# openai/baselines

Hardware: NVIDIA H100
Metric: PPO2 learner env-steps/sec (higher is better)
Workload: dtype f16 operands / f32 accumulate (GAE f64 carry)

## Files before the change

baselines_b200/common/policies.py:

```python
import numpy as np
import torch

from .. import _lib, nn, ops
from . import spaces


RECURRENT_NETWORKS = ("lstm", "cnn_lstm")


class PolicyBuilder:

    def __init__(self, ob_space, ac_space, network, value_network=None, normalize_observations=False,
                 **network_kwargs):
        if callable(network) and not isinstance(network, str):
            raise NotImplementedError("custom network callables build TF graphs in the reference; this learner "
                                      "supports the registry names 'cnn', 'mlp', 'conv_only', 'lstm', 'cnn_lstm'")
        if network in ("lnlstm", "cnn_lnlstm") or (network in RECURRENT_NETWORKS and network_kwargs.get("layer_norm")):
            raise NotImplementedError(f"network={network!r}: layer-normalised LSTMs are not implemented "
                                      "(supported recurrent networks: 'lstm', 'cnn_lstm' without layer_norm)")
        if network in ("impala_cnn", "impala_cnn_lstm"):
            raise NotImplementedError(f"network={network!r}: the IMPALA residual tower is not implemented")
        if value_network not in (None, "shared", "copy"):
            raise NotImplementedError("value_network must be None/'shared'/'copy' (policies.py:154-166)")
        if value_network == "copy" and network in RECURRENT_NETWORKS:
# ... 247 lines not shown
        if self.pd in ("cat", "mcat"):
            ops.cat_step(self.pi_out, self.ld_pi, self.nout, self.v_out, self.ld_v, actions, values, neglogp, B,
                         uniforms=noise, seed=seed, offset_dev=self.rng_ctr, seg_off=self.seg_off)
        elif self.pd == "bern":
            ops.bern_step(self.pi_out, self.ld_pi, self.nout, self.v_out, self.ld_v, actions, values, neglogp, B,
                          uniforms=noise, seed=seed, offset_dev=self.rng_ctr)
        else:
            ops.gauss_step(self.pi_out, self.ld_pi, self.logstd, self.nout, self.v_out, self.ld_v, actions, values,
                           neglogp, B, normals=noise, seed=seed, offset_dev=self.rng_ctr)
        ops.counter_add(self.rng_ctr, 1)

    def _fused_first_wgrad(self, B, alpha):
        tp, tv = self.tower_pi, self.tower_vf
        a, b = tp.fcs[0], tv.fcs[0]
        N2, x, ldx = 2 * a.N, tp._mlp_in, 2 * tp.in_pad
        bn = 256 if N2 == 256 else (128 if N2 > 64 else 64)
        tiles = -(-a.K // 128) * -(-N2 // bn)
        kb = -(-B // 64)
        split = max(1, min(kb // 2 if kb >= 2 else 1, -(-2 * ops.num_sms() // tiles)))
        self.g0cat.zero_()
        for xs in ((x, x[:, a.Kp:]) if a.split_in else (x,)):
            ops.gemm(xs, self.dz0cat, self.g0cat, M=a.K, N=N2, K=B, lda=ldx, ldb=N2, ldc=N2, mn_major=True,
                     mode=ops.MODE_F32_ATOMIC, alpha=alpha * a.in_scale, split_k=split, tag="wgrad.pi+vf/mlp_fc0")
        a.gw.add_(self.g0cat[:, :a.N])
        b.gw.add_(self.g0cat[:, a.N:])
        ops.colsum(tp.dzfc[0], a.gb, B, a.N, N2, alpha=alpha)
        ops.colsum(tv.dzfc[0], b.gb, B, b.N, N2, alpha=alpha)

    def loss_backward(self, x, B, src_idx, actions, returns, old_values, old_neglogp, cliprange, ent_coef, vf_coef,
                      inv_M, seq=None):
        clip_dev = self.clip_dev if cliprange is None else None
        cliprange = 0.0 if cliprange is None else cliprange
        _lib.phase = "@train"
        self.forward(x, B, src_idx, seq=seq)
        if self.pd in ("cat", "mcat"):
            ops.cat_loss(self.pi_out, self.ld_pi, self.nout, self.v_out, self.ld_v, actions, src_idx, returns,
                         old_values, old_neglogp, self.adv_st, cliprange, ent_coef, vf_coef, self.dpi, self.ld_dpi,
                         self.dv, self.ld_dv, self.stats, B, cliprange_dev=clip_dev, seg_off=self.seg_off)
# ... 28 lines not shown
```

baselines_b200/csrc/conv_shift.cu:

```cuda
#include <stdlib.h>

#include <type_traits>

#include "common.cuh"
#include "tc_common.cuh"

namespace b200rl {

static constexpr int SH_BM = 128;
static constexpr int SH_CONSUMER_WARPS = 8;
static constexpr int SH_TMA_WARP = SH_CONSUMER_WARPS;
__host__ __device__ constexpr int sh_threads(bool u8) { return (SH_CONSUMER_WARPS + 1) * 32 + (u8 ? 256 : 0); }
static constexpr int SH_MAX_TAPS = 16;
__host__ __device__ constexpr int sh_arows(int KH) { return KH == 1 ? 160 : 144; }
__host__ __device__ constexpr int sh_stages(int KH) { return KH == 1 ? 6 : 4; }
static constexpr int SH_U8_STAGES = 12;
static constexpr int SH_U8_WRES_BYTES = 16 * 1024;
__host__ __device__ constexpr int sh_wgrad_krows(bool u8) { return u8 ? 128 : 64; }
__host__ __device__ constexpr int sh_wres_bytes(int KH, bool u8) {
  return u8 ? SH_U8_WRES_BYTES : KH == 1 ? 80 * 1024 : 64 * 1024;
}
static constexpr int SH_BAR_BYTES = 512;
__host__ __device__ constexpr int sh_mask_stage_bytes(int BN, bool DACT) { return DACT ? SH_BM * BN / 8 : 0; }
static constexpr int SH_EPI_WARP_BYTES = 16 * 64;
static constexpr int SH_EPI_BYTES = SH_CONSUMER_WARPS * SH_EPI_WARP_BYTES;
static constexpr int SH_WROWS_K = 96;
static constexpr int SH_WABYTES = SH_WROWS_K * 128;
__host__ __device__ constexpr int sh_wgrad_qw(int BN, int KH, bool u8) { return u8 ? 2 : BN == 32 ? 4 : KH == 1 ? 3 : 2; }

static constexpr int SH_ORDER_BAR = 2;
__device__ __forceinline__ void order_wait(int wg) {
  asm volatile("bar.sync %0, %1;" ::"r"(SH_ORDER_BAR + wg), "n"(SH_CONSUMER_WARPS * 32) : "memory");
}
__device__ __forceinline__ void order_pass(int wg) {
  asm volatile("bar.arrive %0, %1;" ::"r"(SH_ORDER_BAR + 1 - wg), "n"(SH_CONSUMER_WARPS * 32) : "memory");
}

struct AddrMap {
  int mode;
  long long sN, sY, sX;
  int Cq, s;
  int Cq_log2, s_log2;
};

__device__ __forceinline__ long long map_rowbase(const AddrMap& a, int n, int y, int x) {
  if (a.mode == 2) {
    const int sm = a.s - 1;
    return (long long)n * a.sN + (long long)(y >> a.s_log2) * a.sY + (long long)(x >> a.s_log2) * a.sX +
           ((((y & sm) << a.s_log2) + (x & sm)) << a.Cq_log2);
  }
  if (a.mode == 1) return (long long)n * a.sN + ((long long)y << a.s_log2) * a.sY + ((long long)x << a.s_log2) * a.sX;
// ... 152 lines not shown
  int Hg, Wg;
  int N;
  int taps;
  int shift[SH_MAX_TAPS];
  int min_shift;
  int vy, vx;
  __half* out;
  AddrMap omap;
  uint16_t* bits_out;
  const uint16_t* saved_bits;
  const float* bias;
  int act, dact;
  float alpha;
  int num_tiles;
};

__device__ __forceinline__ void stmatrix_x4(uint32_t addr, const uint32_t (&r)[4]) {
  asm volatile("stmatrix.sync.aligned.m8n8.x4.shared.b16 [%0], {%1, %2, %3, %4};" ::"r"(addr), "r"(r[0]), "r"(r[1]),
               "r"(r[2]), "r"(r[3])
               : "memory");
}
__device__ __forceinline__ uint4 ld_shared_v4(uint32_t addr) {
  uint4 v;
  asm volatile("ld.shared.v4.b32 {%0,%1,%2,%3}, [%4];" : "=r"(v.x), "=r"(v.y), "=r"(v.z), "=r"(v.w) : "r"(addr) : "memory");
  return v;
}
__device__ __forceinline__ void st_global_v4(void* p, const uint4& v) {
  asm volatile("st.global.v4.b32 [%0], {%1,%2,%3,%4};" ::"l"(p), "r"(v.x), "r"(v.y), "r"(v.z), "r"(v.w) : "memory");
}
__device__ __forceinline__ uint32_t h2_bits(__half2 h) { return *reinterpret_cast<const uint32_t*>(&h); }
__device__ __forceinline__ uint32_t mask_pair(uint32_t b8, int k) {
  const uint32_t b = b8 >> (2 * k);
  return ((b & 1u) | ((b & 2u) << 15)) * 0xffffu;
}

template <int BN, int KH, bool DACT, bool U8>
__global__ void __launch_bounds__(sh_threads(U8), 1)
conv_shift_fwd_kernel(const __grid_constant__ CUtensorMap tmX, const __grid_constant__ CUtensorMap tmW,
                      const __grid_constant__ ShiftParams p) {
  constexpr int SH_ABYTES = sh_arows(KH) * 128;
  constexpr int STAGE_BYTES = KH * SH_ABYTES;
  constexpr int STAGES = U8 ? SH_U8_STAGES : sh_stages(KH);
  using Ring = U8Ring<SH_BM, STAGES>;
  constexpr bool PINGPONG = !(BN == 128 && !DACT);
  constexpr int MH = PINGPONG ? 2 : 1;
  static_assert(PINGPONG || !U8, "the uint8 ring's release rule assumes ping-pong");
  constexpr int A_PITCH = U8 ? SH_BM * 128 : STAGE_BYTES;
  constexpr int A_TOTAL = U8 ? Ring::BYTES : STAGES * STAGE_BYTES;
  extern __shared__ uint8_t smem_raw[];
// ... 77 lines not shown
    }
  } else if (U8 && warp > SH_TMA_WARP) {
    u8_ring_producer<SH_BM, STAGES, 2>(p.u8, p.M, (long long)tile_first * SH_BM + p.min_shift, tile_count, smem,
                                       full_bar, head_bar, empty_bar, warp - (SH_TMA_WARP + 1), lane);
  } else {
    const int wg = __shfl_sync(0xffffffffu, warp >> 2, 0), t = threadIdx.x & 127;
    const int row0 = PINGPONG ? 0 : wg * 64;
    const uint32_t w_base = smem_u32(wres);
    const float lo = (p.act == ACT_RELU) ? 0.0f : -INFINITY;
    const __half2 lo2 = __floats2half2_rn(lo, lo);
    const __half2 zero2 = __floats2half2_rn(0.0f, 0.0f);
    const int er = lane & 15, ep = lane >> 4;
    const int erow = row0 + 16 * (warp & 3) + er;
    uint32_t epi_addr[2];
#pragma unroll
    for (int jj = 0; jj < 2; ++jj)
      epi_addr[jj] = smem_u32(sepi + warp * SH_EPI_WARP_BYTES) + er * 64 + (((2 * jj + ep) ^ ((er >> 1) & 3)) << 4);
    const bool masked = DACT && p.saved_bits != nullptr;
    float acc[MH][BN / 2];
    mbar_wait(w_bar, 0);
    for (int i = PINGPONG ? wg : 0; i < tile_count; i += PINGPONG ? 2 : 1) {
      const int tile = tile_first + i * tile_stride;
      const int s = i % STAGES, s1 = (s + 1 == STAGES) ? 0 : s + 1;
      const uint32_t ph = (uint32_t)(i / STAGES) & 1u;
      mbar_wait(&full_bar[s], ph);
      if (U8) mbar_wait(&head_bar[s1], s1 == 0 ? ph ^ 1 : ph);
      if (PINGPONG && i > 0) order_wait(wg);
      const uint32_t a_base = smem_u32(smem + s * A_PITCH) + (uint32_t)(row0 * 128);
      wgmma_fence();
#pragma unroll 1
      for (int a = 0; a < p.taps; ++a) {
        const uint32_t at = a_base + (uint32_t)p.shift[a] * 128u;
// ... 549 lines not shown
```

baselines_b200/csrc/gemm_wgmma.cu:

```cuda
#include <stdarg.h>
#include <stdio.h>
#include <stdlib.h>

#include <map>
#include <mutex>

#include "common.cuh"
#include "tc_common.cuh"

namespace b200rl {

static constexpr int BM = 128;
static constexpr int BK = 64;
static constexpr int MMA_K = 16;
static constexpr int CONSUMER_WARPS = 8;
static constexpr int NUM_THREADS = CONSUMER_WARPS * 32 + 32;


struct ConvCoords {
  int OW, OH;
  int stride_w, stride_h;
  int lower_w, lower_h;
  int S, taps;
};
// ... 19 lines not shown
  int rm_C, rm_OW, rm_Wg;
  float* ws;
};

template <int BN>
struct Cfg {
  static constexpr int A_BYTES = BM * BK * 2;
  static constexpr int B_BYTES = BN * BK * 2;
  static constexpr int STAGE_BYTES = A_BYTES + B_BYTES;
  static constexpr int STAGES_RAW = (196 * 1024) / STAGE_BYTES;
  static constexpr int STAGES = STAGES_RAW > 8 ? 8 : STAGES_RAW;
  static constexpr int SMEM_BYTES = STAGES * STAGE_BYTES + 1024  + 256 ;
};

static constexpr int BRES_STAGES = 7;
static constexpr int BRES_B_BYTES = 80 * 1024;

__device__ __forceinline__ void gemm_epi_pair(const GemmParams& p, int mode, int split, int row, int col, float v0,
                                              float v1, bool two) {
  if (mode == MODE_F32_ATOMIC) {
    if (p.ws) {
      float* w = p.ws + ((long long)split * p.M + row) * p.N + col;
      w[0] = v0;
      if (two) w[1] = v1;
      return;
    }
    float* out = reinterpret_cast<float*>(p.C) + (long long)row * p.ldc + col;
    atomicAdd(out, v0);
    if (two) atomicAdd(out + 1, v1);
    return;
// ... 41 lines not shown
  }
  int ocol = col;
  if (p.rm_C > 0) {
    const int pix = col / p.rm_C;
    ocol = ((pix / p.rm_OW) * p.rm_Wg + pix % p.rm_OW) * p.rm_C + col % p.rm_C;
  }
  __half* out = C + (long long)row * p.ldc + ocol;
  if (two && p.vec32) {
    *reinterpret_cast<__half2*>(out) = __floats2half2_rn(v0, v1);
  } else {
    out[0] = __float2half_rn(v0);
    if (two) out[1] = __float2half_rn(v1);
  }
}

template <int BN, int CPT, bool MN_MAJOR, bool IM2COL, bool BRES, int TMODE>
__global__ void __launch_bounds__(NUM_THREADS, 1)
gemm_wgmma_kernel(const __grid_constant__ CUtensorMap tmA, const __grid_constant__ CUtensorMap tmB,
                  const GemmParams p) {
  using C_ = Cfg<BN>;
  static_assert(!BRES || (IM2COL && !MN_MAJOR), "resident weights: K-major implicit conv only");
  constexpr int STAGES = BRES ? BRES_STAGES : C_::STAGES;
  constexpr int STAGE_BYTES = BRES ? C_::A_BYTES : C_::STAGE_BYTES;
  constexpr int BROWB = MN_MAJOR ? (BN >= 64 ? 128 : BN * 2) : 0;
  constexpr uint32_t LAYOUT_B = sdesc_layout(BROWB);
  constexpr int BCHUNKS = (BN >= 64) ? BN / 64 : 1;
  constexpr int TPS = BK / CPT;
  constexpr int ROWB = CPT * 2;
  constexpr uint32_t LAYOUT_A = sdesc_layout(ROWB);
  constexpr int A_SUB = BM * ROWB;
  constexpr int B_SUB = BN * ROWB;
  constexpr int A_CHUNK = BK * ROWB;
  constexpr int MCH = BM / CPT;
  extern __shared__ uint8_t smem_raw[];
  uint8_t* smem = reinterpret_cast<uint8_t*>((reinterpret_cast<uintptr_t>(smem_raw) + 1023) & ~uintptr_t(1023));
  uint8_t* bres = smem + STAGES * STAGE_BYTES;
  constexpr int ZT_BYTES = (IM2COL && !MN_MAJOR) ? B_SUB : 0;
  uint8_t* zero_tile = bres + (BRES ? BRES_B_BYTES : 0);
  uint64_t* bars = reinterpret_cast<uint64_t*>(zero_tile + ZT_BYTES);
  uint64_t* full_bar = bars;
  uint64_t* empty_bar = bars + STAGES;
  uint64_t* bres_bar = bars + 2 * STAGES;

  const int warp = threadIdx.x >> 5;
  const int lane = threadIdx.x & 31;
  const int total_work = p.m_tiles * p.n_tiles * p.splits;

  if (threadIdx.x == 0) {
    for (int s = 0; s < STAGES; ++s) {
      mbar_init(&full_bar[s], 1);
      mbar_init(&empty_bar[s], CONSUMER_WARPS);
    }
    mbar_init(bres_bar, 1);
    fence_barrier_init();
  }
  __syncthreads();

  if (warp == CONSUMER_WARPS) {
    if (elect_one()) {
      tma_prefetch_desc(&tmA);
      tma_prefetch_desc(&tmB);
      if (BRES) {
        mbar_arrive_expect_tx(bres_bar, (uint32_t)p.cv.taps * B_SUB);
        for (int g = 0; g < p.cv.taps; ++g) tma_load_2d(bres + g * B_SUB, &tmB, bres_bar, g * CPT, 0);
      }
    }
// ... 55 lines not shown
                                     (uint16_t)(g / p.cv.S));
                } else {
                  tma_load_2d(sa + j * A_CHUNK, &tmA, &full_bar[s], m_tile * BM + j * CPT, kb * BK);
                }
              }
            }
#pragma unroll
            for (int j = 0; j < BCHUNKS; ++j)
              tma_load_2d(sb + j * (BK * BROWB), &tmB, &full_bar[s], n_tile * BN + j * 64, kb * BK);
          }
        }
        __syncwarp();
        if (++s == STAGES) { s = 0; ph ^= 1; }
      }
    }
  } else {
    const int wg = warp >> 2;
    const int t = threadIdx.x & 127;
    const int mode = (TMODE >= 0) ? TMODE : p.mode;
    float acc[BN / 2];
    int s = 0;
    uint32_t ph = 0;
    if (ZT_BYTES > 0) {
      for (int i = threadIdx.x; i < ZT_BYTES / 16; i += CONSUMER_WARPS * 32)
        reinterpret_cast<uint4*>(zero_tile)[i] = make_uint4(0u, 0u, 0u, 0u);
      fence_proxy_async_smem();
      asm volatile("bar.sync 1, %0;" ::"n"(CONSUMER_WARPS * 32) : "memory");
    }
    if (BRES) mbar_wait(bres_bar, 0);
    for (int work = blockIdx.x; work < total_work; work += gridDim.x) {
// ... 193 lines not shown
      const long long r = i / cols;
      out[r * ldo + (i - r * cols)] += t;
    }
    __syncthreads();
  }
}

int sum_partials(const float* ws, int parts, long long rows, int cols, float* out, long long ldo, cudaStream_t stream) {
  const long long n = rows * cols;
  long long blocks = (n + 31) / 32;
  if (blocks > 16LL * num_sms()) blocks = 16LL * num_sms();
  sum_partials_kernel<<<(int)blocks, 256, 0, stream>>>(ws, parts, rows, cols, out, ldo);
  return check_launch("sum_partials_kernel");
}

template <int BN, int CPT, bool MN, bool IM2COL, bool BRES = false, int TMODE = -1>
static int launch(const CUtensorMap& tmA, const CUtensorMap& tmB, const GemmParams& p, int max_ctas,
                  cudaStream_t stream) {
  using C_ = Cfg<BN>;
  constexpr int ZT = (IM2COL && !MN) ? BN * CPT * 2 : 0;
  constexpr int SMEM = (BRES ? (BRES_STAGES * C_::A_BYTES + BRES_B_BYTES + 1024 + 256) : C_::SMEM_BYTES) + ZT;
  static_assert(SMEM <= 227 * 1024, "gemm: shared memory budget");
  static bool attr_set = false;
  auto kern = gemm_wgmma_kernel<BN, CPT, MN, IM2COL, BRES, TMODE>;
  if (!attr_set) {
    cudaError_t e = cudaFuncSetAttribute(kern, cudaFuncAttributeMaxDynamicSharedMemorySize, SMEM);
    if (e != cudaSuccess) {
      set_last_error("cudaFuncSetAttribute(smem=%d): %s", SMEM, cudaGetErrorString(e));
      return B200RL_ERR_CUDA;
    }
    attr_set = true;
  }
  const int total = p.m_tiles * p.n_tiles * p.splits;
  int grid = total < num_sms() ? total : num_sms();
  if (max_ctas > 0 && grid > max_ctas) grid = max_ctas;
  kern<<<grid, NUM_THREADS, SMEM, stream>>>(tmA, tmB, p);
  return check_launch("gemm_wgmma_kernel");
}

static void fill_splits(GemmParams& p, int split_k) {
  int splits = split_k < 1 ? 1 : split_k;
  if (splits > p.kb_total) splits = p.kb_total;
  p.kb_per_split = ceil_div(p.kb_total, splits);
  p.splits = ceil_div(p.kb_total, p.kb_per_split);
}

static int gemm_dispatch(int BN, int mn_major, int mode, const CUtensorMap& tmA, const CUtensorMap& tmB,
                         const GemmParams& p, int max_ctas, cudaStream_t stream) {
  if (mn_major) {
    B200RL_REQUIRE(mode == MODE_F32_ATOMIC, "gemm: the MN-major (wgrad) layout uses the fp32 atomic epilogue");
    if (BN == 64) return launch<64, 64, true, false, false, MODE_F32_ATOMIC>(tmA, tmB, p, max_ctas, stream);
    if (BN == 256) return launch<256, 64, true, false, false, MODE_F32_ATOMIC>(tmA, tmB, p, max_ctas, stream);
    return launch<128, 64, true, false, false, MODE_F32_ATOMIC>(tmA, tmB, p, max_ctas, stream);
  }
#define GEMM_KMAJOR(bn)                                                                                         \
  switch (mode) {                                                                                               \
    case MODE_F16_ACT: return launch<bn, 64, false, false, false, MODE_F16_ACT>(tmA, tmB, p, max_ctas, stream);   \
    case MODE_F32_STORE: return launch<bn, 64, false, false, false, MODE_F32_STORE>(tmA, tmB, p, max_ctas, stream); \
    case MODE_F16_DACT: return launch<bn, 64, false, false, false, MODE_F16_DACT>(tmA, tmB, p, max_ctas, stream);  \
    default: return launch<bn, 64, false, false, false, MODE_F32_ATOMIC>(tmA, tmB, p, max_ctas, stream);          \
  }
  switch (BN) {
    case 32: GEMM_KMAJOR(32)
    case 64: GEMM_KMAJOR(64)
    case 128: GEMM_KMAJOR(128)
    default: GEMM_KMAJOR(256)
  }
#undef GEMM_KMAJOR
}

template <int CPT, bool MN>
static int launch_conv(int BN, bool bres, const CUtensorMap& tmA, const CUtensorMap& tmB, const GemmParams& p,
                       cudaStream_t st) {
  if (MN) {
    switch (BN) {
      case 32: return launch<32, CPT, MN, true>(tmA, tmB, p, 0, st);
      case 64: return launch<64, CPT, MN, true>(tmA, tmB, p, 0, st);
      case 128: return launch<128, CPT, MN, true>(tmA, tmB, p, 0, st);
      default: break;
    }
  } else if (bres) {
// ... 28 lines not shown
  B200RL_REQUIRE(rm_C == 0 || (rm_C % 16 == 0 && rm_OW > 0 && rm_Wg >= rm_OW && (mode == MODE_F16_ACT || mode == MODE_F16_DACT)),
                 "gemm: bad column remap");
  B200RL_REQUIRE(M > 0 && N > 0 && K > 0, "gemm: bad shape M=%d N=%d K=%d", M, N, K);
  B200RL_REQUIRE((lda % 8) == 0 && (ldb % 8) == 0, "gemm: lda/ldb must be multiples of 8 fp16 (16 B): %lld %lld", lda,
                 ldb);
  B200RL_REQUIRE((reinterpret_cast<uintptr_t>(A) & 15) == 0 && (reinterpret_cast<uintptr_t>(B) & 15) == 0,
                 "gemm: operands must be 16-byte aligned");
  B200RL_REQUIRE(mode >= 0 && mode <= 3, "gemm: bad mode %d", mode);
  B200RL_REQUIRE(mode != MODE_F16_DACT || saved != nullptr || saved_bits != nullptr,
                 "gemm: MODE_F16_DACT needs the saved activation (or its bit mask)");
  B200RL_REQUIRE(saved_bits == nullptr || (mode == MODE_F16_DACT && act == ACT_RELU && (ld_saved % 16) == 0 && (N % 16) == 0),
                 "gemm: saved_bits is a ReLU mask for MODE_F16_DACT with ld_saved and N multiples of 16");

  int BN;
  if (mn_major) BN = (N > 128 && N % 256 == 0) ? 256 : (N > 64) ? 128 : 64;
  else BN = (N > 128 && (N % 256 == 0)) ? 256 : (N > 64) ? 128 : (N > 32) ? 64 : 32;

  GemmParams p = {};
  p.M = M; p.N = N; p.K = K;
  p.m_tiles = ceil_div(M, BM);
  p.n_tiles = ceil_div(N, BN);
  p.kb_total = ceil_div(K, BK);
  B200RL_REQUIRE(split_k <= 1 || mode == MODE_F32_ATOMIC, "gemm: split_k needs the fp32 atomic epilogue");
  fill_splits(p, split_k);
  p.C = C; p.ldc = ldc; p.bias = bias; p.saved = reinterpret_cast<const __half*>(saved); p.ld_saved = ld_saved;
  p.saved_bits = reinterpret_cast<const uint16_t*>(saved_bits);
  p.alpha = alpha; p.mode = mode; p.act = act;
  p.rm_C = rm_C; p.rm_OW = rm_OW; p.rm_Wg = rm_Wg;
  p.vec32 = ((ldc & 15) == 0) && ((reinterpret_cast<uintptr_t>(C) & 31) == 0) && (rm_C == 0 || (rm_C & 15) == 0) &&
            (!saved || (((ld_saved & 15) == 0) && ((reinterpret_cast<uintptr_t>(saved) & 31) == 0)));
  B200RL_REQUIRE(saved_bits == nullptr || p.vec32, "gemm: saved_bits needs 32-byte aligned 16-column output chunks");

  CUtensorMap tmA, tmB;
  int rc;
  if (!mn_major) {
    if ((rc = make_tmap(&tmA, A, M, K, lda, BK, BM)) != 0) return rc;
    if ((rc = make_tmap(&tmB, B, N, K, ldb, BK, BN)) != 0) return rc;
  } else {
    if ((rc = make_tmap(&tmA, A, K, M, lda, 64, BK)) != 0) return rc;
    if ((rc = make_tmap(&tmB, B, K, N, ldb, 64, BK)) != 0) return rc;
  }
  if (mode == MODE_F32_ATOMIC && p.splits > 1) {
    if ((p.ws = det_workspace((size_t)p.splits * M * N, stream)) == nullptr) return B200RL_ERR_CUDA;
  }
  rc = gemm_dispatch(BN, mn_major, mode, tmA, tmB, p, max_ctas, stream);
  if (rc == B200RL_OK && p.ws) rc = sum_partials(p.ws, p.splits, M, N, reinterpret_cast<float*>(C), ldc, stream);
  return rc;
}

extern "C" int b200rl_conv_gemm(const void* x, long long B, int H, int W, int C, int R, int S, int stride_h,
                                int stride_w, int pad_h, int pad_w, int OH, int OW, const void* Wt_or_dz, long long ldb,
                                void* out, long long ldc, const float* bias, const void* saved, long long ld_saved,
                                int N, int kind, int mode, int act, float alpha, int split_k, int sh_H, int sh_W,
                                int sh_C, int sh_s, void* stream_) {
  cudaStream_t stream = static_cast<cudaStream_t>(stream_);
  B200RL_REQUIRE(x && Wt_or_dz && out && B > 0, "conv_gemm: null operand");
  B200RL_REQUIRE(C == 16 || C == 32 || C == 64, "conv_gemm: channels per tap must be 16, 32 or 64 (got %d)", C);
  B200RL_REQUIRE((reinterpret_cast<uintptr_t>(x) & 15) == 0 && (ldb % 8) == 0, "conv_gemm: alignment");
  B200RL_REQUIRE(kind == 0 || kind == 1, "conv_gemm: bad kind");
  const int taps = R * S;
// ... 29 lines not shown
    fill_splits(p, 1);
    if ((rc = make_tmap_im2col(&tmA, x, B, H, W, C, lower_w, lower_h, upper_w, upper_h, stride_w, stride_h, BM)) != 0)
      return rc;
    if ((rc = make_tmap(&tmB, Wt_or_dz, N, (long long)taps * C, ldb, C, BN)) != 0) return rc;
    const bool bres = (p.n_tiles == 1) && ((long long)taps * BN * C * 2 <= BRES_B_BYTES) && (split_k != -1);
    if (C == 64) return launch_conv<64, false>(BN, bres, tmA, tmB, p, stream);
    if (C == 32) return launch_conv<32, false>(BN, bres, tmA, tmB, p, stream);
    return launch_conv<16, false>(BN, bres, tmA, tmB, p, stream);
  }
  B200RL_REQUIRE(mode == MODE_F32_ATOMIC, "conv_gemm: wgrad needs the fp32 atomic epilogue");
  const int BN = (N > 64) ? 128 : (N > 32) ? 64 : 32;
  p.M = taps * C; p.N = N; p.K = (int)rows;
  p.m_tiles = ceil_div(p.M, BM);
  p.n_tiles = ceil_div(N, BN);
  p.kb_total = ceil_div(p.K, BK);
  fill_splits(p, split_k);
  if ((rc = make_tmap_im2col(&tmA, x, B, H, W, C, lower_w, lower_h, upper_w, upper_h, stride_w, stride_h, BK)) != 0)
    return rc;
  if ((rc = make_tmap(&tmB, Wt_or_dz, rows, N, ldb, BN < 64 ? BN : 64, BK)) != 0) return rc;
  if (p.splits > 1) {
    if ((p.ws = det_workspace((size_t)p.splits * p.M * p.N, stream)) == nullptr) return B200RL_ERR_CUDA;
  }
  rc = (C == 64) ? launch_conv<64, true>(BN, false, tmA, tmB, p, stream)
     : (C == 32) ? launch_conv<32, true>(BN, false, tmA, tmB, p, stream)
                 : launch_conv<16, true>(BN, false, tmA, tmB, p, stream);
  if (rc == B200RL_OK && p.ws) rc = sum_partials(p.ws, p.splits, p.M, p.N, reinterpret_cast<float*>(out), ldc, stream);
  return rc;
}
```

baselines_b200/csrc/tc_common.cuh:

```cuda
#pragma once
#include "common.cuh"
#include "wgmma.cuh"

namespace b200rl {

enum : int { MODE_F16_ACT = 0, MODE_F32_STORE = 1, MODE_F32_ATOMIC = 2, MODE_F16_DACT = 3, MODE_F16_SHUFFLE = 4 };
enum : int { ACT_NONE = 0, ACT_RELU = 1, ACT_TANH = 2 };

__host__ __device__ constexpr uint32_t sdesc_layout(int row_bytes) {
  return row_bytes == 128 ? 1u : row_bytes == 64 ? 2u : 3u;
}
__device__ __forceinline__ uint64_t make_sdesc(uint32_t saddr, uint32_t lbo_bytes, uint32_t sbo_bytes, uint32_t layout) {
  uint64_t d = 0;
  d |= (uint64_t)((saddr & 0x3FFFFu) >> 4);
  d |= (uint64_t)((lbo_bytes >> 4) & 0x3FFFu) << 16;
  d |= (uint64_t)((sbo_bytes >> 4) & 0x3FFFu) << 32;
  d |= (uint64_t)layout << 62;
  return d;
}

__device__ __forceinline__ int acc_row(int t, int e) { return 16 * (t >> 5) + ((t & 31) >> 2) + 8 * ((e >> 1) & 1); }
__device__ __forceinline__ int acc_col(int t, int e) { return 8 * (e >> 2) + 2 * (t & 3) + (e & 1); }

__device__ __forceinline__ void tma_load_im2col_4d(void* smem_dst, const CUtensorMap* tmap, uint64_t* bar, int c, int w,
// ... 4 lines not shown
      ::"r"(smem_u32(smem_dst)), "l"(tmap), "r"(smem_u32(bar)), "r"(c), "r"(w), "r"(h), "r"(n), "h"(off_w), "h"(off_h)
      : "memory");
}

__device__ __forceinline__ float apply_act(float x, int act) {
  if (act == ACT_RELU) return fmaxf(x, 0.0f);
  if (act == ACT_TANH) return tanhf(x);
  return x;
}
__device__ __forceinline__ float act_grad_from_saved(float h, int act) {
  if (act == ACT_RELU) return h > 0.0f ? 1.0f : 0.0f;
  if (act == ACT_TANH) return 1.0f - h * h;
  return 1.0f;
}

int make_tmap_2d_f16(CUtensorMap* tm, const void* ptr, long long rows, long long cols, long long ld, int box_cols,
                     int box_rows);

}
```

baselines_b200/nn.py:

```python
import functools
import math
from collections import OrderedDict, namedtuple

import numpy as np
import torch

from . import ops

NATURE_CONVS = (("c1", 32, 8, 4), ("c2", 64, 4, 2), ("c3", 64, 3, 1))


def _pad8(n):
    return (n + 7) // 8 * 8


def ortho_init(shape, scale, rng=np.random):
    shape = tuple(shape)
    flat = shape if len(shape) == 2 else (int(np.prod(shape[:-1])), shape[-1])
    a = rng.normal(0.0, 1.0, flat)
    u, _, v = np.linalg.svd(a, full_matrices=False)
    q = (u if u.shape == flat else v).reshape(shape)
    return (scale * q[:shape[0], :shape[1]]).astype(np.float32)


# ... 125 lines not shown
        self.w_fwd = torch.zeros(self.N, self.Kf, dtype=torch.float16, device=dev)
        self.w_bwd = torch.zeros(self.K, self.Np, dtype=torch.float16, device=dev)

    def cast_jobs(self):
        jobs = [ops.CastJob(self.w, self.K, self.N, self.w_bwd, self.Np, self.w_fwd, self.Kf, self.in_scale)]
        if self.split_in:
            jobs.append(ops.CastJob(self.w, self.K, self.N, None, 0, self.w_fwd[:, self.Kp:], self.Kf, self.in_scale))
        return jobs

    def forward(self, x, ldx, M, out, ldo, mode=ops.MODE_F16_ACT, act=None):
        K = self.Kp + self.K if self.split_in else self.K
        ops.gemm(x, self.w_fwd, out, M=M, N=self.N, K=K, lda=ldx, ldb=self.Kf, ldc=ldo, bias=self.b,
                 mode=mode, act=self.act if act is None else act, tag="fwd." + self.name)

    def wgrad(self, x, ldx, dz, lddz, M, alpha):
        bn = 256 if (self.N > 128 and self.N % 256 == 0) else (128 if self.N > 64 else 64)
        tiles = -(-self.K // 128) * -(-self.N // bn)
        kb = -(-M // 64)
        split = max(1, min(kb // 2 if kb >= 2 else 1, -(-2 * ops.num_sms() // tiles)))
        ops.gemm(x, dz, self.gw, M=self.K, N=self.N, K=M, lda=ldx, ldb=lddz, ldc=self.N, mn_major=True,
                 mode=ops.MODE_F32_ATOMIC, alpha=alpha * self.in_scale, split_k=split, tag="wgrad." + self.name)
        if self.split_in:
            ops.gemm(x[:, self.Kp:], dz, self.gw, M=self.K, N=self.N, K=M, lda=ldx, ldb=lddz, ldc=self.N,
                     mn_major=True, mode=ops.MODE_F32_ATOMIC, alpha=alpha * self.in_scale, split_k=split,
                     tag="wgrad." + self.name)
        ops.colsum(dz, self.gb, M, self.N, lddz, alpha=alpha)

    def dgrad(self, dz, lddz, M, out, ldo, saved=None, ld_saved=0, act=ops.ACT_NONE, remap=(0, 0, 0), saved_bits=None):
        if saved_bits is not None and act == ops.ACT_RELU:
            ops.gemm(dz, self.w_bwd, out, M=M, N=self.K, K=self.N, lda=lddz, ldb=self.Np, ldc=ldo, saved_bits=saved_bits,
                     ld_saved=ld_saved, mode=ops.MODE_F16_DACT, act=act, tag="dgrad." + self.name, remap=remap)
        elif saved is None or act == ops.ACT_NONE:
            ops.gemm(dz, self.w_bwd, out, M=M, N=self.K, K=self.N, lda=lddz, ldb=self.Np, ldc=ldo,
                     mode=ops.MODE_F16_ACT, act=ops.ACT_NONE, tag="dgrad." + self.name, remap=remap)
        else:
            ops.gemm(dz, self.w_bwd, out, M=M, N=self.K, K=self.N, lda=lddz, ldb=self.Np, ldc=ldo, saved=saved,
                     ld_saved=ld_saved, mode=ops.MODE_F16_DACT, act=act, tag="dgrad." + self.name, remap=remap)


# ... 76 lines not shown
                                   device=self.store.device)

    def operand_launches(self):
        if self.wdg is None:
            return []
        return [functools.partial(ops.dgrad_weights, self.w, self.wdg, self.rf, self.rf, self.C, self.nf, self.stride,
                                  self.ld_wdg)]

    def fwd_implicit(self, x, B, out):
        H, W, C, R, S, sh, sw, pt, pl = self.geom
        ops.conv_gemm(x, B, H, W, C, R, S, sh, sw, pt, pl, self.OH, self.OW, self.w_fwd, self.Kp, out, self.nf,
                      self.nf, 0, ops.MODE_F16_ACT, act=self.act, bias=self.b, tag="fwd." + self.name)

    def wgrad_implicit(self, x, dz, B, alpha):
        H, W, C, R, S, sh, sw, pt, pl = self.geom
        tiles = -(-self.K // 128)
        rows = B * self.P
        split = max(1, min((rows // 64) // 2 if rows >= 128 else 1, -(-2 * ops.num_sms() // tiles)))
        ops.conv_gemm(x, B, H, W, C, R, S, sh, sw, pt, pl, self.OH, self.OW, dz, self.nf, self.gw, self.nf, self.nf, 1,
                      ops.MODE_F32_ATOMIC, alpha=alpha * self.in_scale, split_k=split, tag="wgrad." + self.name)
        ops.colsum(dz, self.gb, rows, self.nf, self.nf, alpha=alpha)

    def dgrad_implicit(self, dz, B, saved_in, dx, act):
        s, An = self.stride, self.An
        G_h, G_w = -(-self.H // s), -(-self.W // s)
        ops.conv_gemm(dz, B, self.OH, self.OW, self.nf, An, An, 1, 1, An - 1, An - 1, G_h, G_w, self.wdg, self.ld_wdg,
                      dx, 0, s * s * self.C, 0, ops.MODE_F16_SHUFFLE, act=act, saved=saved_in,
                      shuffle=(self.H, self.W, self.C, s), tag="dgrad." + self.name)


LSTM_SIZES = (64, 128)

Seq = namedtuple("Seq", "T B masks mask_idx state state_idx state_out")
Seq.__doc__ = """How the rows of one LSTM pass form sequences: T time-major steps of B environments (row t*B + b); masks
uint8 "done before step t" of row r at masks[mask_idx[r]] (mask_idx None: masks[r]); environment b starts from row
# ... 39 lines not shown
    def forward(self, x, ldx, seq, train=True):
        H, rows = self.H, seq.T * seq.B
        self.wx.forward(x, ldx, rows, self.xg, 4 * H, mode=ops.MODE_F32_STORE, act=ops.ACT_NONE)
        ops.lstm_seq_fwd(self.xg, 4 * H, self.wh16, seq.masks, seq.state, self.h, H, seq.T, seq.B, H,
                         mask_idx=seq.mask_idx, state_idx=seq.state_idx, state_out=seq.state_out,
                         hprev_out=self.hprev if train else None, gates_out=self.xg if train else None,
                         c_out=self.c if train else None)
        self._x, self._ldx, self._seq = x, ldx, seq
        return self.h, H

    def backward(self, alpha, dx=None, ldo=0, saved=None, ld_saved=0, act=ops.ACT_NONE):
        H, seq = self.H, self._seq
        rows = seq.T * seq.B
        ops.lstm_seq_bwd(self.dh, H, self.xg, self.c, seq.masks, seq.state, self.whT16, self.dz, 4 * H, seq.T, seq.B, H,
                         mask_idx=seq.mask_idx, state_idx=seq.state_idx)
        tiles = -(-H // 128) * -(-4 * H // 256)
        kb = -(-rows // 64)
        split = max(1, min(kb // 2 if kb >= 2 else 1, -(-2 * ops.num_sms() // tiles)))
        ops.gemm(self.hprev, self.dz, self.gwh, M=H, N=4 * H, K=rows, lda=H, ldb=4 * H, ldc=4 * H, mn_major=True,
                 mode=ops.MODE_F32_ATOMIC, alpha=alpha, split_k=split, tag="wgrad.lstm/wh")
        self.wx.wgrad(self._x, self._ldx, self.dz, 4 * H, rows, alpha)
        if dx is not None:
            self.wx.dgrad(self.dz, 4 * H, rows, dx, ldo, saved=saved, ld_saved=ld_saved, act=act)


ConvLayerPlan = namedtuple("ConvLayerPlan", "path s2d geom implicit_dgrad kx")
ConvLayerPlan.__doc__ = """How one conv layer runs.  path: "shift" (csrc/conv_shift.cu), "implicit" (TMA im2col GEMM over the
input viewed as geom = (H, W, C, R, S, stride_h, stride_w, pad_t, pad_l)) or "explicit" (im2col + GEMM).  s2d: the
layer reads its input space-to-depth'ed (and its master weight rows are stored in that order).  implicit_dgrad: the
data gradient is one implicit GEMM with the pixel-shuffle epilogue instead of GEMM + col2im.  kx: taps per filter row
the shift-GEMM weight gradient folds into one pass."""
ConvStackPlan = namedtuple("ConvStackPlan", "shift fused_u8 layers")
ConvStackPlan.__doc__ = """shift: every layer runs as shift-GEMM, and every layer writes its 1-bit ReLU mask, which the next
data gradient (or fc1's) reads.  fused_u8: the first shift layer reads the uint8 frames itself."""

# ... 417 lines not shown
```

Before: 1.188 million.

## Add ping-pong consumer warpgroup schedule for fp16-epilogue K-major GEMMs

Adds a ping-pong variant of the wgmma GEMM kernel. The two consumer warpgroups take alternating tiles, use ordered barriers to take turns on the MMA, and each runs its fp16 epilogue through its own stmatrix staging area, so one group's epilogue overlaps the other's math. This variant is chosen when the tile count exceeds the grid. K-major BN=256 tiles are dropped in favour of at most 128 for all non-wgrad GEMMs. The split-k heuristic moves from Python into the C++ side (split_k=0 means auto), and the shared epilogue helpers move into tc_common.cuh. The risks are extra shared memory for the epilogue and more, smaller tiles where BN=256 was used before.

After: 1.269 million (median of 6 runs). 1.07x the previous value.

```diff
diff --git a/baselines_b200/common/policies.py b/baselines_b200/common/policies.py
--- a/baselines_b200/common/policies.py
+++ b/baselines_b200/common/policies.py
@@ -285,14 +285,10 @@
         tp, tv = self.tower_pi, self.tower_vf
         a, b = tp.fcs[0], tv.fcs[0]
         N2, x, ldx = 2 * a.N, tp._mlp_in, 2 * tp.in_pad
-        bn = 256 if N2 == 256 else (128 if N2 > 64 else 64)
-        tiles = -(-a.K // 128) * -(-N2 // bn)
-        kb = -(-B // 64)
-        split = max(1, min(kb // 2 if kb >= 2 else 1, -(-2 * ops.num_sms() // tiles)))
         self.g0cat.zero_()
         for xs in ((x, x[:, a.Kp:]) if a.split_in else (x,)):
             ops.gemm(xs, self.dz0cat, self.g0cat, M=a.K, N=N2, K=B, lda=ldx, ldb=N2, ldc=N2, mn_major=True,
-                     mode=ops.MODE_F32_ATOMIC, alpha=alpha * a.in_scale, split_k=split, tag="wgrad.pi+vf/mlp_fc0")
+                     mode=ops.MODE_F32_ATOMIC, alpha=alpha * a.in_scale, split_k=0, tag="wgrad.pi+vf/mlp_fc0")
         a.gw.add_(self.g0cat[:, :a.N])
         b.gw.add_(self.g0cat[:, a.N:])
         ops.colsum(tp.dzfc[0], a.gb, B, a.N, N2, alpha=alpha)
diff --git a/baselines_b200/csrc/conv_shift.cu b/baselines_b200/csrc/conv_shift.cu
--- a/baselines_b200/csrc/conv_shift.cu
+++ b/baselines_b200/csrc/conv_shift.cu
@@ -22,19 +22,12 @@
 }
 static constexpr int SH_BAR_BYTES = 512;
 __host__ __device__ constexpr int sh_mask_stage_bytes(int BN, bool DACT) { return DACT ? SH_BM * BN / 8 : 0; }
-static constexpr int SH_EPI_WARP_BYTES = 16 * 64;
-static constexpr int SH_EPI_BYTES = SH_CONSUMER_WARPS * SH_EPI_WARP_BYTES;
+static constexpr int SH_EPI_BYTES = SH_CONSUMER_WARPS * EPI_WARP_BYTES;
 static constexpr int SH_WROWS_K = 96;
 static constexpr int SH_WABYTES = SH_WROWS_K * 128;
 __host__ __device__ constexpr int sh_wgrad_qw(int BN, int KH, bool u8) { return u8 ? 2 : BN == 32 ? 4 : KH == 1 ? 3 : 2; }
 
-static constexpr int SH_ORDER_BAR = 2;
-__device__ __forceinline__ void order_wait(int wg) {
-  asm volatile("bar.sync %0, %1;" ::"r"(SH_ORDER_BAR + wg), "n"(SH_CONSUMER_WARPS * 32) : "memory");
-}
-__device__ __forceinline__ void order_pass(int wg) {
-  asm volatile("bar.arrive %0, %1;" ::"r"(SH_ORDER_BAR + 1 - wg), "n"(SH_CONSUMER_WARPS * 32) : "memory");
-}
+static_assert(SH_CONSUMER_WARPS * 32 == 256, "order_wait / order_pass join 256 consumer threads");
 
 struct AddrMap {
   int mode;
@@ -217,25 +210,6 @@
   float alpha;
   int num_tiles;
 };
-
-__device__ __forceinline__ void stmatrix_x4(uint32_t addr, const uint32_t (&r)[4]) {
-  asm volatile("stmatrix.sync.aligned.m8n8.x4.shared.b16 [%0], {%1, %2, %3, %4};" ::"r"(addr), "r"(r[0]), "r"(r[1]),
-               "r"(r[2]), "r"(r[3])
-               : "memory");
-}
-__device__ __forceinline__ uint4 ld_shared_v4(uint32_t addr) {
-  uint4 v;
-  asm volatile("ld.shared.v4.b32 {%0,%1,%2,%3}, [%4];" : "=r"(v.x), "=r"(v.y), "=r"(v.z), "=r"(v.w) : "r"(addr) : "memory");
-  return v;
-}
-__device__ __forceinline__ void st_global_v4(void* p, const uint4& v) {
-  asm volatile("st.global.v4.b32 [%0], {%1,%2,%3,%4};" ::"l"(p), "r"(v.x), "r"(v.y), "r"(v.z), "r"(v.w) : "memory");
-}
-__device__ __forceinline__ uint32_t h2_bits(__half2 h) { return *reinterpret_cast<const uint32_t*>(&h); }
-__device__ __forceinline__ uint32_t mask_pair(uint32_t b8, int k) {
-  const uint32_t b = b8 >> (2 * k);
-  return ((b & 1u) | ((b & 2u) << 15)) * 0xffffu;
-}
 
 template <int BN, int KH, bool DACT, bool U8>
 __global__ void __launch_bounds__(sh_threads(U8), 1)
@@ -343,8 +317,7 @@
     const int erow = row0 + 16 * (warp & 3) + er;
     uint32_t epi_addr[2];
 #pragma unroll
-    for (int jj = 0; jj < 2; ++jj)
-      epi_addr[jj] = smem_u32(sepi + warp * SH_EPI_WARP_BYTES) + er * 64 + (((2 * jj + ep) ^ ((er >> 1) & 3)) << 4);
+    for (int jj = 0; jj < 2; ++jj) epi_addr[jj] = epi_lane_addr(smem_u32(sepi + warp * EPI_WARP_BYTES), lane, jj);
     const bool masked = DACT && p.saved_bits != nullptr;
     float acc[MH][BN / 2];
     mbar_wait(w_bar, 0);
diff --git a/baselines_b200/csrc/gemm_wgmma.cu b/baselines_b200/csrc/gemm_wgmma.cu
--- a/baselines_b200/csrc/gemm_wgmma.cu
+++ b/baselines_b200/csrc/gemm_wgmma.cu
@@ -57,6 +57,8 @@
 };
 
 static constexpr int BRES_STAGES = 7;
+static constexpr int BAR_BYTES = 256;
+static constexpr int EPI_BYTES = CONSUMER_WARPS * EPI_WARP_BYTES;
 static constexpr int BRES_B_BYTES = 80 * 1024;
 
 __device__ __forceinline__ void gemm_epi_pair(const GemmParams& p, int mode, int split, int row, int col, float v0,
@@ -128,12 +130,14 @@
   }
 }
 
-template <int BN, int CPT, bool MN_MAJOR, bool IM2COL, bool BRES, int TMODE>
+template <int BN, int CPT, bool MN_MAJOR, bool IM2COL, bool BRES, int TMODE, bool PP>
 __global__ void __launch_bounds__(NUM_THREADS, 1)
 gemm_wgmma_kernel(const __grid_constant__ CUtensorMap tmA, const __grid_constant__ CUtensorMap tmB,
                   const GemmParams p) {
   using C_ = Cfg<BN>;
   static_assert(!BRES || (IM2COL && !MN_MAJOR), "resident weights: K-major implicit conv only");
+  static_assert(!PP || (!MN_MAJOR && !IM2COL && CPT == 64 && BN <= 128 && (TMODE == MODE_F16_ACT || TMODE == MODE_F16_DACT)),
+                "ping-pong: plain K-major GEMMs with an fp16 epilogue, 2 x BN/2 accumulators per thread, at most 128");
   constexpr int STAGES = BRES ? BRES_STAGES : C_::STAGES;
   constexpr int STAGE_BYTES = BRES ? C_::A_BYTES : C_::STAGE_BYTES;
   constexpr int BROWB = MN_MAJOR ? (BN >= 64 ? 128 : BN * 2) : 0;
@@ -163,7 +167,7 @@
   if (threadIdx.x == 0) {
     for (int s = 0; s < STAGES; ++s) {
       mbar_init(&full_bar[s], 1);
-      mbar_init(&empty_bar[s], CONSUMER_WARPS);
+      mbar_init(&empty_bar[s], PP ? 4 : CONSUMER_WARPS);
     }
     mbar_init(bres_bar, 1);
     fence_barrier_init();
@@ -249,6 +253,134 @@
         if (++s == STAGES) { s = 0; ph ^= 1; }
       }
     }
+  } else if (PP) {
+    const int wg = __shfl_sync(0xffffffffu, warp >> 2, 0);
+    const int t = threadIdx.x & 127;
+    const int mode = (TMODE >= 0) ? TMODE : p.mode;
+    const uint32_t epi_base = smem_u32(reinterpret_cast<uint8_t*>(bars) + BAR_BYTES) + warp * EPI_WARP_BYTES;
+    const int er = lane & 15, ep = lane >> 4;
+    float acc[2][BN / 2];
+    int s = 0;
+    uint32_t ph = 0;
+    int i = 0;
+    for (int work = blockIdx.x; work < total_work; work += gridDim.x, ++i) {
+      const int n_tile = work % p.n_tiles;
+      const int t2 = work / p.n_tiles;
+      const int m_tile = t2 % p.m_tiles;
+      const int split = t2 / p.m_tiles;
+      const int kb0 = split * p.kb_per_split;
+      const int kb1 = min(kb0 + p.kb_per_split, p.kb_total);
+      if ((i & 1) != wg) {
+        s += kb1 - kb0;
+        ph ^= (uint32_t)(s / STAGES) & 1u;
+        s %= STAGES;
+        continue;
+      }
+      if (i > 0) order_wait(wg);
+      int prev = -1;
+      for (int kb = kb0; kb < kb1; ++kb) {
+        mbar_wait(&full_bar[s], ph);
+        const uint32_t st = smem_u32(smem + s * STAGE_BYTES);
+        wgmma_fence();
+#pragma unroll
+        for (int k = 0; k < BK / MMA_K; ++k) {
+          const uint64_t bdesc = make_sdesc(st + C_::A_BYTES + k * (MMA_K * 2), 16, 8 * ROWB, LAYOUT_A);
+#pragma unroll
+          for (int mh = 0; mh < 2; ++mh) {
+            const uint64_t adesc = make_sdesc(st + mh * 64 * ROWB + k * (MMA_K * 2), 16, 8 * ROWB, LAYOUT_A);
+            wgmma_f16<BN, 0, 0>(acc[mh], adesc, bdesc, (kb > kb0 || k > 0) ? 1u : 0u);
+          }
+        }
+        wgmma_commit();
+        wgmma_wait<1>();
+        if (prev >= 0) {
+          __syncwarp();
+          if (lane == 0) mbar_arrive(&empty_bar[prev]);
+        }
+        prev = s;
+        if (++s == STAGES) { s = 0; ph ^= 1; }
+      }
+      if (work + (int)gridDim.x < total_work) order_pass(wg);
+      wgmma_wait<0>();
+      __syncwarp();
+      if (lane == 0) mbar_arrive(&empty_bar[prev]);
+
+      const int col0 = n_tile * BN;
+#pragma unroll
+      for (int mh = 0; mh < 2; ++mh) {
+        const int frow = m_tile * BM + mh * 64 + 16 * (warp & 3);
+        const bool bits = mode == MODE_F16_DACT && p.saved_bits != nullptr;
+        const int orow = frow + er;
+        __half* C = reinterpret_cast<__half*>(p.C) + (long long)orow * p.ldc;
+#pragma unroll
+        for (int ps = 0; ps < BN / 32; ++ps) {
+          uint32_t mw[2] = {0u, 0u};
+          if (bits) {
+#pragma unroll
+            for (int jj = 0; jj < 2; ++jj) {
+              const int c16 = col0 + 32 * ps + 16 * jj;
+              if (orow < p.M && c16 < p.N) mw[jj] = __ldg(p.saved_bits + (((long long)orow * p.ld_saved + c16) >> 4));
+            }
+          }
+#pragma unroll
+          for (int jj = 0; jj < 2; ++jj) {
+            const int b = 2 * (2 * ps + jj);
+            uint32_t r[4];
+#pragma unroll
+            for (int k = 0; k < 4; ++k) {
+              const int e = 4 * (b + (k >> 1)) + 2 * (k & 1);
+              const int row = frow + ((t & 31) >> 2) + 8 * (k & 1);
+              const int col = col0 + 8 * (b + (k >> 1)) + 2 * (t & 3);
+              float v0 = acc[mh][e] * p.alpha, v1 = acc[mh][e + 1] * p.alpha;
+              if (mode == MODE_F16_ACT) {
+                if (p.bias) {
+                  v0 += col < p.N ? __ldg(p.bias + col) : 0.0f;
+                  v1 += col + 1 < p.N ? __ldg(p.bias + col + 1) : 0.0f;
+                }
+                v0 = apply_act(v0, p.act);
+                v1 = apply_act(v1, p.act);
+              } else if (!bits && row < p.M) {
+                const long long so = (long long)row * p.ld_saved + col;
+                if (col < p.N) v0 *= act_grad_from_saved(__half2float(p.saved[so]), p.act);
+                if (col + 1 < p.N) v1 *= act_grad_from_saved(__half2float(p.saved[so + 1]), p.act);
+              }
+              r[k] = h2_bits(__floats2half2_rn(v0, v1));
+            }
+            stmatrix_x4(epi_lane_addr(epi_base, lane, jj), r);
+          }
+          __syncwarp();
+#pragma unroll
+          for (int jj = 0; jj < 2; ++jj) {
+            const int c16 = col0 + 32 * ps + 16 * jj;
+            const int col = c16 + 8 * ep;
+            uint4 v = ld_shared_v4(epi_lane_addr(epi_base, lane, jj));
+            if (bits) {
+              const uint32_t b8 = (mw[jj] >> (8 * ep)) & 0xffu;
+              v.x &= mask_pair(b8, 0);
+              v.y &= mask_pair(b8, 1);
+              v.z &= mask_pair(b8, 2);
+              v.w &= mask_pair(b8, 3);
+            }
+            if (orow < p.M && col < p.N) {
+              int ocol = col;
+              if (p.rm_C > 0) {
+                const int pix = c16 / p.rm_C;
+                ocol = ((pix / p.rm_OW) * p.rm_Wg + pix % p.rm_OW) * p.rm_C + c16 % p.rm_C + 8 * ep;
+              }
+              if (p.vec32 && col + 8 <= p.N) {
+                st_global_v4(C + ocol, v);
+              } else {
+                const __half* h = reinterpret_cast<const __half*>(&v);
+#pragma unroll
+                for (int q = 0; q < 8; ++q)
+                  if (col + q < p.N) C[ocol + q] = h[q];
+              }
+            }
+          }
+          __syncwarp();
+        }
+      }
+    }
   } else {
     const int wg = warp >> 2;
     const int t = threadIdx.x & 127;
@@ -472,15 +604,16 @@
   return check_launch("sum_partials_kernel");
 }
 
-template <int BN, int CPT, bool MN, bool IM2COL, bool BRES = false, int TMODE = -1>
+template <int BN, int CPT, bool MN, bool IM2COL, bool BRES = false, int TMODE = -1, bool PP = false>
 static int launch(const CUtensorMap& tmA, const CUtensorMap& tmB, const GemmParams& p, int max_ctas,
                   cudaStream_t stream) {
   using C_ = Cfg<BN>;
   constexpr int ZT = (IM2COL && !MN) ? BN * CPT * 2 : 0;
-  constexpr int SMEM = (BRES ? (BRES_STAGES * C_::A_BYTES + BRES_B_BYTES + 1024 + 256) : C_::SMEM_BYTES) + ZT;
+  constexpr int EPI = PP ? EPI_BYTES : 0;
+  constexpr int SMEM = (BRES ? (BRES_STAGES * C_::A_BYTES + BRES_B_BYTES + 1024 + 256) : C_::SMEM_BYTES) + ZT + EPI;
   static_assert(SMEM <= 227 * 1024, "gemm: shared memory budget");
   static bool attr_set = false;
-  auto kern = gemm_wgmma_kernel<BN, CPT, MN, IM2COL, BRES, TMODE>;
+  auto kern = gemm_wgmma_kernel<BN, CPT, MN, IM2COL, BRES, TMODE, PP>;
   if (!attr_set) {
     cudaError_t e = cudaFuncSetAttribute(kern, cudaFuncAttributeMaxDynamicSharedMemorySize, SMEM);
     if (e != cudaSuccess) {
@@ -496,6 +629,12 @@
   return check_launch("gemm_wgmma_kernel");
 }
 
+static int auto_splits(int tiles, int kb) {
+  const int cap = kb >= 2 ? kb / 2 : 1;
+  const int want = ceil_div(2 * num_sms(), tiles);
+  return want < cap ? (want > 1 ? want : 1) : cap;
+}
+
 static void fill_splits(GemmParams& p, int split_k) {
   int splits = split_k < 1 ? 1 : split_k;
   if (splits > p.kb_total) splits = p.kb_total;
@@ -503,7 +642,7 @@
   p.splits = ceil_div(p.kb_total, p.kb_per_split);
 }
 
-static int gemm_dispatch(int BN, int mn_major, int mode, const CUtensorMap& tmA, const CUtensorMap& tmB,
+static int gemm_dispatch(int BN, int mn_major, int mode, bool pingpong, const CUtensorMap& tmA, const CUtensorMap& tmB,
                          const GemmParams& p, int max_ctas, cudaStream_t stream) {
   if (mn_major) {
     B200RL_REQUIRE(mode == MODE_F32_ATOMIC, "gemm: the MN-major (wgrad) layout uses the fp32 atomic epilogue");
@@ -511,18 +650,21 @@
     if (BN == 256) return launch<256, 64, true, false, false, MODE_F32_ATOMIC>(tmA, tmB, p, max_ctas, stream);
     return launch<128, 64, true, false, false, MODE_F32_ATOMIC>(tmA, tmB, p, max_ctas, stream);
   }
-#define GEMM_KMAJOR(bn)                                                                                         \
-  switch (mode) {                                                                                               \
-    case MODE_F16_ACT: return launch<bn, 64, false, false, false, MODE_F16_ACT>(tmA, tmB, p, max_ctas, stream);   \
-    case MODE_F32_STORE: return launch<bn, 64, false, false, false, MODE_F32_STORE>(tmA, tmB, p, max_ctas, stream); \
-    case MODE_F16_DACT: return launch<bn, 64, false, false, false, MODE_F16_DACT>(tmA, tmB, p, max_ctas, stream);  \
-    default: return launch<bn, 64, false, false, false, MODE_F32_ATOMIC>(tmA, tmB, p, max_ctas, stream);          \
+#define GEMM_KMAJOR(bn)                                                                                              \
+  switch (mode) {                                                                                                    \
+    case MODE_F16_ACT:                                                                                               \
+      return pingpong ? launch<bn, 64, false, false, false, MODE_F16_ACT, true>(tmA, tmB, p, max_ctas, stream)      \
+                      : launch<bn, 64, false, false, false, MODE_F16_ACT>(tmA, tmB, p, max_ctas, stream);           \
+    case MODE_F32_STORE: return launch<bn, 64, false, false, false, MODE_F32_STORE>(tmA, tmB, p, max_ctas, stream);  \
+    case MODE_F32_ATOMIC: return launch<bn, 64, false, false, false, MODE_F32_ATOMIC>(tmA, tmB, p, max_ctas, stream);\
+    default:                                                                                                         \
+      return pingpong ? launch<bn, 64, false, false, false, MODE_F16_DACT, true>(tmA, tmB, p, max_ctas, stream)     \
+                      : launch<bn, 64, false, false, false, MODE_F16_DACT>(tmA, tmB, p, max_ctas, stream);          \
   }
   switch (BN) {
     case 32: GEMM_KMAJOR(32)
     case 64: GEMM_KMAJOR(64)
-    case 128: GEMM_KMAJOR(128)
-    default: GEMM_KMAJOR(256)
+    default: GEMM_KMAJOR(128)
   }
 #undef GEMM_KMAJOR
 }
@@ -581,7 +723,7 @@
 
   int BN;
   if (mn_major) BN = (N > 128 && N % 256 == 0) ? 256 : (N > 64) ? 128 : 64;
-  else BN = (N > 128 && (N % 256 == 0)) ? 256 : (N > 64) ? 128 : (N > 32) ? 64 : 32;
+  else BN = (N > 64) ? 128 : (N > 32) ? 64 : 32;
 
   GemmParams p = {};
   p.M = M; p.N = N; p.K = K;
@@ -589,6 +731,8 @@
   p.n_tiles = ceil_div(N, BN);
   p.kb_total = ceil_div(K, BK);
   B200RL_REQUIRE(split_k <= 1 || mode == MODE_F32_ATOMIC, "gemm: split_k needs the fp32 atomic epilogue");
+  B200RL_REQUIRE(split_k >= 0, "gemm: bad split_k %d", split_k);
+  if (split_k == 0) split_k = (mode == MODE_F32_ATOMIC) ? auto_splits(p.m_tiles * p.n_tiles, p.kb_total) : 1;
   fill_splits(p, split_k);
   p.C = C; p.ldc = ldc; p.bias = bias; p.saved = reinterpret_cast<const __half*>(saved); p.ld_saved = ld_saved;
   p.saved_bits = reinterpret_cast<const uint16_t*>(saved_bits);
@@ -610,7 +754,12 @@
   if (mode == MODE_F32_ATOMIC && p.splits > 1) {
     if ((p.ws = det_workspace((size_t)p.splits * M * N, stream)) == nullptr) return B200RL_ERR_CUDA;
   }
-  rc = gemm_dispatch(BN, mn_major, mode, tmA, tmB, p, max_ctas, stream);
+  long long grid = (long long)p.m_tiles * p.n_tiles * p.splits;
+  if (grid > num_sms()) grid = num_sms();
+  if (max_ctas > 0 && grid > max_ctas) grid = max_ctas;
+  const bool pingpong = !mn_major && (mode == MODE_F16_ACT || mode == MODE_F16_DACT) &&
+                        (long long)p.m_tiles * p.n_tiles * p.splits > grid;
+  rc = gemm_dispatch(BN, mn_major, mode, pingpong, tmA, tmB, p, max_ctas, stream);
   if (rc == B200RL_OK && p.ws) rc = sum_partials(p.ws, p.splits, M, N, reinterpret_cast<float*>(C), ldc, stream);
   return rc;
 }
@@ -670,6 +819,7 @@
   p.m_tiles = ceil_div(p.M, BM);
   p.n_tiles = ceil_div(N, BN);
   p.kb_total = ceil_div(p.K, BK);
+  if (split_k == 0) split_k = auto_splits(p.m_tiles * p.n_tiles, (int)(rows / BK));
   fill_splits(p, split_k);
   if ((rc = make_tmap_im2col(&tmA, x, B, H, W, C, lower_w, lower_h, upper_w, upper_h, stride_w, stride_h, BK)) != 0)
     return rc;
diff --git a/baselines_b200/csrc/tc_common.cuh b/baselines_b200/csrc/tc_common.cuh
--- a/baselines_b200/csrc/tc_common.cuh
+++ b/baselines_b200/csrc/tc_common.cuh
@@ -42,6 +42,38 @@
   return 1.0f;
 }
 
+static constexpr int ORDER_BAR = 2;
+__device__ __forceinline__ void order_wait(int wg) {
+  asm volatile("bar.sync %0, %1;" ::"r"(ORDER_BAR + wg), "n"(256) : "memory");
+}
+__device__ __forceinline__ void order_pass(int wg) {
+  asm volatile("bar.arrive %0, %1;" ::"r"(ORDER_BAR + 1 - wg), "n"(256) : "memory");
+}
+
+static constexpr int EPI_WARP_BYTES = 16 * 64;
+__device__ __forceinline__ uint32_t epi_lane_addr(uint32_t warp_scratch, int lane, int jj) {
+  const int er = lane & 15, ep = lane >> 4;
+  return warp_scratch + er * 64 + (((2 * jj + ep) ^ ((er >> 1) & 3)) << 4);
+}
+__device__ __forceinline__ void stmatrix_x4(uint32_t addr, const uint32_t (&r)[4]) {
+  asm volatile("stmatrix.sync.aligned.m8n8.x4.shared.b16 [%0], {%1, %2, %3, %4};" ::"r"(addr), "r"(r[0]), "r"(r[1]),
+               "r"(r[2]), "r"(r[3])
+               : "memory");
+}
+__device__ __forceinline__ uint4 ld_shared_v4(uint32_t addr) {
+  uint4 v;
+  asm volatile("ld.shared.v4.b32 {%0,%1,%2,%3}, [%4];" : "=r"(v.x), "=r"(v.y), "=r"(v.z), "=r"(v.w) : "r"(addr) : "memory");
+  return v;
+}
+__device__ __forceinline__ void st_global_v4(void* p, const uint4& v) {
+  asm volatile("st.global.v4.b32 [%0], {%1,%2,%3,%4};" ::"l"(p), "r"(v.x), "r"(v.y), "r"(v.z), "r"(v.w) : "memory");
+}
+__device__ __forceinline__ uint32_t h2_bits(__half2 h) { return *reinterpret_cast<const uint32_t*>(&h); }
+__device__ __forceinline__ uint32_t mask_pair(uint32_t b8, int k) {
+  const uint32_t b = b8 >> (2 * k);
+  return ((b & 1u) | ((b & 2u) << 15)) * 0xffffu;
+}
+
 int make_tmap_2d_f16(CUtensorMap* tm, const void* ptr, long long rows, long long cols, long long ld, int box_cols,
                      int box_rows);
 
diff --git a/baselines_b200/nn.py b/baselines_b200/nn.py
--- a/baselines_b200/nn.py
+++ b/baselines_b200/nn.py
@@ -163,15 +163,11 @@
                  mode=mode, act=self.act if act is None else act, tag="fwd." + self.name)
 
     def wgrad(self, x, ldx, dz, lddz, M, alpha):
-        bn = 256 if (self.N > 128 and self.N % 256 == 0) else (128 if self.N > 64 else 64)
-        tiles = -(-self.K // 128) * -(-self.N // bn)
-        kb = -(-M // 64)
-        split = max(1, min(kb // 2 if kb >= 2 else 1, -(-2 * ops.num_sms() // tiles)))
         ops.gemm(x, dz, self.gw, M=self.K, N=self.N, K=M, lda=ldx, ldb=lddz, ldc=self.N, mn_major=True,
-                 mode=ops.MODE_F32_ATOMIC, alpha=alpha * self.in_scale, split_k=split, tag="wgrad." + self.name)
+                 mode=ops.MODE_F32_ATOMIC, alpha=alpha * self.in_scale, split_k=0, tag="wgrad." + self.name)
         if self.split_in:
             ops.gemm(x[:, self.Kp:], dz, self.gw, M=self.K, N=self.N, K=M, lda=ldx, ldb=lddz, ldc=self.N,
-                     mn_major=True, mode=ops.MODE_F32_ATOMIC, alpha=alpha * self.in_scale, split_k=split,
+                     mn_major=True, mode=ops.MODE_F32_ATOMIC, alpha=alpha * self.in_scale, split_k=0,
                      tag="wgrad." + self.name)
         ops.colsum(dz, self.gb, M, self.N, lddz, alpha=alpha)
 
@@ -278,11 +274,9 @@
 
     def wgrad_implicit(self, x, dz, B, alpha):
         H, W, C, R, S, sh, sw, pt, pl = self.geom
-        tiles = -(-self.K // 128)
         rows = B * self.P
-        split = max(1, min((rows // 64) // 2 if rows >= 128 else 1, -(-2 * ops.num_sms() // tiles)))
         ops.conv_gemm(x, B, H, W, C, R, S, sh, sw, pt, pl, self.OH, self.OW, dz, self.nf, self.gw, self.nf, self.nf, 1,
-                      ops.MODE_F32_ATOMIC, alpha=alpha * self.in_scale, split_k=split, tag="wgrad." + self.name)
+                      ops.MODE_F32_ATOMIC, alpha=alpha * self.in_scale, split_k=0, tag="wgrad." + self.name)
         ops.colsum(dz, self.gb, rows, self.nf, self.nf, alpha=alpha)
 
     def dgrad_implicit(self, dz, B, saved_in, dx, act):
@@ -352,11 +346,8 @@
         rows = seq.T * seq.B
         ops.lstm_seq_bwd(self.dh, H, self.xg, self.c, seq.masks, seq.state, self.whT16, self.dz, 4 * H, seq.T, seq.B, H,
                          mask_idx=seq.mask_idx, state_idx=seq.state_idx)
-        tiles = -(-H // 128) * -(-4 * H // 256)
-        kb = -(-rows // 64)
-        split = max(1, min(kb // 2 if kb >= 2 else 1, -(-2 * ops.num_sms() // tiles)))
         ops.gemm(self.hprev, self.dz, self.gwh, M=H, N=4 * H, K=rows, lda=H, ldb=4 * H, ldc=4 * H, mn_major=True,
-                 mode=ops.MODE_F32_ATOMIC, alpha=alpha, split_k=split, tag="wgrad.lstm/wh")
+                 mode=ops.MODE_F32_ATOMIC, alpha=alpha, split_k=0, tag="wgrad.lstm/wh")
         self.wx.wgrad(self._x, self._ldx, self.dz, 4 * H, rows, alpha)
         if dx is not None:
             self.wx.dgrad(self.dz, 4 * H, rows, dx, ldo, saved=saved, ld_saved=ld_saved, act=act)
```
